# V-DETR/V-DETR

Measured on AMD Instinct MI355X. Metric: scenes/sec (train fwd+bwd) 40k-pt ScanNet, higher is better.
Workload: dtype f32

## Files before the change

v-detr_amd/csrc/attn_bwd_box4.hip:

```cpp
#include "attn_common.h"

#include <stdlib.h>

namespace vdetr {

typedef f32x4 __attribute__((may_alias)) b4_rec4_t;
typedef float __attribute__((may_alias)) b4_rec1_t;
typedef int __attribute__((may_alias)) b4_reci_t;
typedef unsigned __attribute__((may_alias)) b4_recu_t;

constexpr int kB4Waves = 16;
constexpr int kB4Threads = kB4Waves * kWave;
constexpr int kB4T = 10;
constexpr int kB4RecBytes = 64;
constexpr int kB4StripBytes = kWave * kB4RecBytes + (kWave + 4) * 4 + 2 * kWave * 4;
constexpr int kB4TableWords = 4 * kB4T * kB4T * kB4T * 4;

size_t attn_bwd_box4_lds_bytes() { return (size_t)kB4TableWords * 4 + (size_t)kB4Waves * kB4StripBytes + 64; }

__device__ __forceinline__ unsigned b4_wave_incl_scan(unsigned v) {
  v += (unsigned)__builtin_amdgcn_update_dpp(0, (int)v, 0x111, 0xF, 0xF, false);
  v += (unsigned)__builtin_amdgcn_update_dpp(0, (int)v, 0x112, 0xF, 0xF, false);
  v += (unsigned)__builtin_amdgcn_update_dpp(0, (int)v, 0x114, 0xF, 0xF, false);
  v += (unsigned)__builtin_amdgcn_update_dpp(0, (int)v, 0x118, 0xF, 0xF, false);
  v += (unsigned)__builtin_amdgcn_update_dpp(0, (int)v, kDppRowBcast15, 0xA, 0xF, false);
  v += (unsigned)__builtin_amdgcn_update_dpp(0, (int)v, kDppRowBcast31, 0xC, 0xF, false);
  return v;
}
__device__ __forceinline__ int b4_round(float x) {
  int r;
  asm("v_cvt_rpi_i32_f32 %0, %1" : "=v"(r) : "v"(x));
  return r;
}

template <bool NEAREST>
__global__ __launch_bounds__(kB4Threads) void attn_bwd_box4_kernel(AttnParams P) {
  constexpr int T = kB4T, T3 = T * T * T;
  if (P.bwd_aux[4] != 0 || P.bwd_aux[5] == 0) return;
  extern __shared__ __attribute__((aligned(16))) float smem[];
  char* lds = reinterpret_cast<char*>(smem);
  int* tab = reinterpret_cast<int*>(lds);
  const int tid = threadIdx.x, lane = tid & 63;
  const int wv = __builtin_amdgcn_readfirstlane(tid >> 6);
  char* rec = lds + (size_t)kB4TableWords * 4 + (size_t)wv * kB4StripBytes;
  char* sigs = rec + kWave * kB4RecBytes;
  char* wcnt = sigs + (kWave + 4) * 4;
  char* wfirst = wcnt + kWave * 4;
  unsigned* misc = reinterpret_cast<unsigned*>(lds + (size_t)kB4TableWords * 4 + (size_t)kB4Waves * kB4StripBytes);
  const int part = blockIdx.x & 1, nwg = gridDim.x >> 1;
  const int items = P.B * P.nQ;
  for (int i = tid; i < kB4TableWords; i += kB4Threads) tab[i] = 0;
  for (int i = lane; i < kB4StripBytes / 4; i += kWave) reinterpret_cast<b4_recu_t*>(rec)[i] = 0u;
  const int per_wg = (items + nwg - 1) / nwg;
  const int cap = bwd_query_cap(per_wg);
  float fix_scale = 1.f, fix_inv = 1.f;
  {
    const float dmax = sqrtf(__uint_as_float(P.bwd_aux[0]) * __uint_as_float(P.bwd_aux[1]));
    const float bound = 2.f * P.drop_scale * dmax * (float)cap;
    if (bound > 0.f && bound < INFINITY) {
      const int e = 30 - (int)ceilf(__log2f(bound) + 1e-3f);
      fix_scale = ldexpf(1.f, e);
      fix_inv = ldexpf(1.f, -e);
    }
  }
  unsigned* counter = const_cast<unsigned*>(P.bwd_aux) + 2 + part;
  if (tid == 0) misc[0] = atomicAdd(counter, 1u);
  __syncthreads();
  int item = (int)misc[0];
  int taken = 1;

  const int kk = lane >> 4, c15 = lane & 15;
  const int a_off = (((c15 >> 2) & 1) ^ kk) * 16 + (c15 & 3) * 4;
  const int b_offx = (2 ^ kk) * 16 + (2 * ((c15 >> 2) & 1) + (c15 >> 3)) * 4, b_offd = (3 ^ kk) * 16 + (c15 & 3) * 4;
  const int o_xi = c15 >> 3;
  const int o_lane = (((kk & 1) * T + ((c15 >> 2) & 1)) * 4 + (c15 & 3)) * 4;
  const int o_c0 = (o_xi ? 3 : 0) * T3 * 16 + o_lane, o_c1 = (o_xi ? 2 : 1) * T3 * 16 + o_lane;
  const int o_xshift = 20 + 4 * o_xi;

  using rsrc_t = __amdgpu_buffer_rsrc_t;
  auto make_rsrc = [](const void* p, unsigned bytes) {
    return __builtin_amdgcn_make_buffer_rsrc(const_cast<void*>(p), 0, (int)bytes, 0x00020000);
  };
  auto ldf = [](rsrc_t r, int voff, int soff) {
    return __builtin_bit_cast(float, __builtin_amdgcn_raw_buffer_load_b32(r, voff, soff, 0));
  };
  auto uni = [](float x) { return __int_as_float(__builtin_amdgcn_readfirstlane(__float_as_int(x))); };
  const int rowbytes = P.nK * 4;
  const bool rot = P.cos_sin != nullptr;
  const int nchunks = (P.nK + kWave - 1) / kWave;
  struct Ops { float d[4], kx, ky, kz; };
  auto fetch = [&](rsrc_t rd, rsrc_t rx, int chunk, Ops& o) {
    const int key = chunk * kWave + lane;
#pragma unroll
    for (int h = 0; h < 4; ++h)
      o.d[h] = __builtin_bit_cast(float, __builtin_amdgcn_raw_buffer_load_b32(rd, key * 4, h * rowbytes, kStreamAux));
    o.kx = ldf(rx, key * 12, 0); o.ky = ldf(rx, key * 12 + 4, 0); o.kz = ldf(rx, key * 12 + 8, 0);
  };

  int slot_of_next = 1;
  while (item < items) {
    int drawn = items;
    if (tid == 0 && taken < cap) asm volatile("global_atomic_add %0, %1, %2, off sc0\n\ts_nop 3" : "=&v"(drawn) : "v"(counter), "v"(1) : "memory");
    const int b = item / P.nQ;
    const rsrc_t rd = make_rsrc(P.dprob + (size_t)item * 4 * P.nK, 4u * rowbytes);
    const rsrc_t rx = make_rsrc(P.xyz + (size_t)b * P.nK * 3, 3u * rowbytes);
    Ops ops;
    fetch(rd, rx, wv, ops);
    const float* vp = P.vertices + (size_t)item * 24;
    const float bx0 = vp[0], bx1 = vp[6], by0 = vp[1], by1 = vp[4], bz = vp[part * 12 + 2];
    float X0 = uni(bx0), X1 = uni(bx1), Y0 = uni(by0), Y1 = uni(by1), Zp = uni(bz);
    float rc = 1.f, rs = 0.f;
    if (rot) {
      rc = uni(P.cos_sin[(size_t)item * 2]); rs = uni(P.cos_sin[(size_t)item * 2 + 1]);
      float ex = uni(vp[9]) - X0, ey = uni(vp[10]) - Y0;
      rpe_rotate(ex, ey, rc, rs);
      float fx = uni(vp[3]) - X0, fy = uni(vp[4]) - Y0;
      rpe_rotate(fx, fy, rc, rs);
      X1 = ex; Y1 = fy;
    }
    for (int chunk = wv; chunk < nchunks; chunk += kB4Waves) {
      const int ns = min(kWave, P.nK - chunk * kWave);
      const bool valid = lane < ns;
      float dx0 = X0 - ops.kx, dy0 = Y0 - ops.ky, dx1 = X1 - ops.kx, dy1 = Y1 - ops.ky;
      if (rot) {
        rpe_rotate(dx0, dy0, rc, rs);
        dx1 = dx0 + X1; dy1 = dy0 + Y1;
      }
      const AxisTap az = rpe_axis<NEAREST>(Zp - ops.kz, P);
      const AxisTap ay0 = rpe_axis<NEAREST>(dy0, P), ay1 = rpe_axis<NEAREST>(dy1, P);
      const AxisTap ax0 = rpe_axis<NEAREST>(dx0, P), ax1 = rpe_axis<NEAREST>(dx1, P);
      const int zrow = az.base * (T * T);
      const int J = (zrow + ay0.base * T) | ((zrow + ay1.base * T) << 10) | (ax0.base << 20) | (ax1.base << 24);
      const unsigned hsh = ((unsigned)J * 0x9E3779B1u) >> 26;
      const float u0 = az.wa * ay0.wa, u1 = az.wa * ay1.wa, u2 = az.wb * ay0.wa, u3 = az.wb * ay1.wa;
      const float u4 = az.wa * ay0.wb, u5 = az.wa * ay1.wb, u6 = az.wb * ay0.wb, u7 = az.wb * ay1.wb;
      const float d0 = ops.d[0] * fix_scale, d1 = ops.d[1] * fix_scale, d2 = ops.d[2] * fix_scale, d3 = ops.d[3] * fix_scale;
      if (chunk + kB4Waves < nchunks) fetch(rd, rx, chunk + kB4Waves, ops);
      __builtin_amdgcn_wave_barrier();
      unsigned rank = 0;
      if (valid) rank = __hip_atomic_fetch_add(reinterpret_cast<b4_recu_t*>(wcnt) + hsh, 1u, __ATOMIC_RELAXED, __HIP_MEMORY_SCOPE_WAVEFRONT);
      __builtin_amdgcn_wave_barrier();
      const unsigned cnt = reinterpret_cast<const b4_recu_t*>(wcnt)[lane];
      const unsigned incl = b4_wave_incl_scan(cnt);
      reinterpret_cast<b4_recu_t*>(wfirst)[lane] = incl - cnt;
      reinterpret_cast<b4_recu_t*>(wcnt)[lane] = 0u;
      __builtin_amdgcn_wave_barrier();
      if (valid) {
        const unsigned slot = reinterpret_cast<const b4_recu_t*>(wfirst)[hsh] + rank;
        char* mine = rec + slot * kB4RecBytes;
        const unsigned sw = (slot & 3u) << 4;
        *reinterpret_cast<b4_rec4_t*>(mine + sw) = f32x4{u0, u1, u2, u3};
        *reinterpret_cast<b4_rec4_t*>(mine + (sw ^ 16u)) = f32x4{u4, u5, u6, u7};
        *reinterpret_cast<b4_rec4_t*>(mine + (sw ^ 32u)) = f32x4{ax0.wa, ax1.wa, ax0.wb, ax1.wb};
        *reinterpret_cast<b4_rec4_t*>(mine + (sw ^ 48u)) = f32x4{d0, d1, d2, d3};
        reinterpret_cast<b4_reci_t*>(sigs)[slot] = J;
      }
      __builtin_amdgcn_wave_barrier();
      const int Jm = valid ? reinterpret_cast<const b4_reci_t*>(sigs)[lane] : -1;
      const int Jn = lane + 1 < ns ? reinterpret_cast<const b4_reci_t*>(sigs)[lane + 1] : -2;
      const char* rq = rec + kk * kB4RecBytes;
      float u[kWave / 4], t[kWave / 4];
#pragma unroll
      for (int i = 0; i < kWave / 4; ++i) {
        u[i] = *reinterpret_cast<const b4_rec1_t*>(rq + i * 4 * kB4RecBytes + a_off);
        t[i] = *reinterpret_cast<const b4_rec1_t*>(rq + i * 4 * kB4RecBytes + b_offx) *
               *reinterpret_cast<const b4_rec1_t*>(rq + i * 4 * kB4RecBytes + b_offd);
      }
      const unsigned long long emask = __ballot(valid && Jm != Jn);
      f32x4 acc = {0.f, 0.f, 0.f, 0.f};
      auto flush = [&](int slot) {
        const int Jg = __builtin_amdgcn_readlane(Jm, slot);
        const int cell0 = Jg & 1023, cell1 = (Jg >> 10) & 1023;
        if (lane < 32) {
          const int xb = (int)__builtin_amdgcn_ubfe((unsigned)Jg, (unsigned)o_xshift, 4u);
          char* bin0 = reinterpret_cast<char*>(tab) + ((cell0 + xb) << 4) + o_c0;
          char* bin1 = reinterpret_cast<char*>(tab) + ((cell1 + xb) << 4) + o_c1;
          atomicAdd(reinterpret_cast<int*>(bin0), b4_round(acc[0]));
          atomicAdd(reinterpret_cast<int*>(bin1), b4_round(acc[1]));
          atomicAdd(reinterpret_cast<int*>(bin0 + T * T * 16), b4_round(acc[2]));
          atomicAdd(reinterpret_cast<int*>(bin1 + T * T * 16), b4_round(acc[3]));
        }
        acc = f32x4{0.f, 0.f, 0.f, 0.f};
      };
      if (ns == kWave) {
#pragma unroll
        for (int i = 0; i < kWave / 4; ++i) {
          const unsigned eb = (unsigned)(emask >> (4 * i)) & 0xFu;
          if (eb == 0u) {
            acc = __builtin_amdgcn_mfma_f32_16x16x4f32(u[i], t[i], acc, 0, 0, 0);
          } else if (eb == 8u) {
            acc = __builtin_amdgcn_mfma_f32_16x16x4f32(u[i], t[i], acc, 0, 0, 0);
            flush(4 * i + 3);
          } else {
            const int e0 = __builtin_ctz(eb);
            const bool head = kk <= e0;
            acc = __builtin_amdgcn_mfma_f32_16x16x4f32(head ? u[i] : 0.f, t[i], acc, 0, 0, 0);
            flush(4 * i + e0);
            unsigned rest = eb & (eb - 1u);
            if ((rest & 7u) == 0u) {
              acc = __builtin_amdgcn_mfma_f32_16x16x4f32(head ? 0.f : u[i], t[i], acc, 0, 0, 0);
              if (rest) flush(4 * i + 3);
            } else {
              int s = e0 + 1;
              do {
                const int e = rest ? __builtin_ctz(rest) : 3;
                acc = __builtin_amdgcn_mfma_f32_16x16x4f32(kk >= s && kk <= e ? u[i] : 0.f, t[i], acc, 0, 0, 0);
                if (rest) {
                  flush(4 * i + e);
                  rest &= rest - 1u;
                }
                s = e + 1;
              } while (s < 4);
            }
          }
        }
      } else {
        for (int i = 0; 4 * i < ns; ++i) {
          unsigned eb = (unsigned)(emask >> (4 * i)) & 0xFu;
          const int nq = min(4, ns - 4 * i);
          const float ui = *reinterpret_cast<const b4_rec1_t*>(rq + i * 4 * kB4RecBytes + a_off);
          const float ti = *reinterpret_cast<const b4_rec1_t*>(rq + i * 4 * kB4RecBytes + b_offx) *
                           *reinterpret_cast<const b4_rec1_t*>(rq + i * 4 * kB4RecBytes + b_offd);
          int s = 0;
          do {
            const int e = eb ? __builtin_ctz(eb) : 3;
            acc = __builtin_amdgcn_mfma_f32_16x16x4f32(kk >= s && kk <= e ? ui : 0.f, ti, acc, 0, 0, 0);
            if (eb) {
              flush(4 * i + e);
              eb &= eb - 1u;
            }
            s = e + 1;
          } while (s < nq);
        }
      }
    }
    if (tid == 0) {
      asm volatile("s_waitcnt vmcnt(0)" ::: "memory");
      misc[slot_of_next] = (unsigned)drawn;
    }
    asm volatile("s_waitcnt lgkmcnt(0)\n\ts_barrier" ::: "memory");
    item = (int)misc[slot_of_next];
    slot_of_next ^= 3;
    if (taken < cap) ++taken;
  }
  __syncthreads();
  float* dst = P.dtable_part + (size_t)blockIdx.x * kB4TableWords;
  for (int i = tid; i < kB4TableWords; i += kB4Threads) dst[i] = (float)tab[i] * fix_inv;
}

int launch_attn_bwd_box4(const AttnParams& P, int grid, hipStream_t st) {
  const size_t lds = attn_bwd_box4_lds_bytes();
  if (P.rpe_nearest) {
    if (int e = set_lds(attn_bwd_box4_kernel<true>, lds, "attn_bwd_box4")) return e;
    hipLaunchKernelGGL(attn_bwd_box4_kernel<true>, dim3(grid), dim3(kB4Threads), lds, st, P);
    return check_launch("attn_bwd_box4");
  }
  if (int e = set_lds(attn_bwd_box4_kernel<false>, lds, "attn_bwd_box4")) return e;
  hipLaunchKernelGGL(attn_bwd_box4_kernel<false>, dim3(grid), dim3(kB4Threads), lds, st, P);
  return check_launch("attn_bwd_box4");
}

}
```

Baseline: 158.6.

## Split segmented MFMA reduction across accumulator halves using segment-parity masks

Uses a prefix-parity word over segment boundaries so that alternating segments are accumulated into different output halves of the 16x16 MFMA. A per-lane keep mask on the A operand routes each segment, which lets most quads run a single MFMA instead of one per segment. Flushes then come from whichever half owns the segment. This reduces the number of MFMAs and serialised branches in the full-wave path. The cost is extra bit-manipulation and more complex correctness reasoning; the partial-wave path is restricted to the lower half.

```diff
diff --git a/v-detr_amd/csrc/attn_bwd_box4.hip b/v-detr_amd/csrc/attn_bwd_box4.hip
--- a/v-detr_amd/csrc/attn_bwd_box4.hip
+++ b/v-detr_amd/csrc/attn_bwd_box4.hip
@@ -1,4 +1,5 @@
 #include "attn_common.h"
+#include "box4_walk.h"
 
 #include <stdlib.h>
 
@@ -167,11 +168,12 @@
                *reinterpret_cast<const b4_rec1_t*>(rq + i * 4 * kB4RecBytes + b_offd);
       }
       const unsigned long long emask = __ballot(valid && Jm != Jn);
+      const unsigned long long par = b4_parity_word(emask);
       f32x4 acc = {0.f, 0.f, 0.f, 0.f};
-      auto flush = [&](int slot) {
+      auto flush_half = [&](int slot, int half) {
         const int Jg = __builtin_amdgcn_readlane(Jm, slot);
         const int cell0 = Jg & 1023, cell1 = (Jg >> 10) & 1023;
-        if (lane < 32) {
+        if ((lane >> 5) == half) {
           const int xb = (int)__builtin_amdgcn_ubfe((unsigned)Jg, (unsigned)o_xshift, 4u);
           char* bin0 = reinterpret_cast<char*>(tab) + ((cell0 + xb) << 4) + o_c0;
           char* bin1 = reinterpret_cast<char*>(tab) + ((cell1 + xb) << 4) + o_c1;
@@ -179,46 +181,31 @@
           atomicAdd(reinterpret_cast<int*>(bin1), b4_round(acc[1]));
           atomicAdd(reinterpret_cast<int*>(bin0 + T * T * 16), b4_round(acc[2]));
           atomicAdd(reinterpret_cast<int*>(bin1 + T * T * 16), b4_round(acc[3]));
+          acc = f32x4{0.f, 0.f, 0.f, 0.f};
         }
-        acc = f32x4{0.f, 0.f, 0.f, 0.f};
       };
+      auto flush = [&](int slot) { flush_half(slot, b4_half_of_slot(par, slot)); };
       if (ns == kWave) {
+        const unsigned long long keep = b4_keep_word(par, c15, kk);
+        const unsigned keep_lo = (unsigned)keep, keep_hi = (unsigned)(keep >> 32);
 #pragma unroll
         for (int i = 0; i < kWave / 4; ++i) {
+          const int km = __builtin_amdgcn_sbfe((int)(i < 8 ? keep_lo : keep_hi), (unsigned)(4 * i & 31), 1u);
+          const float ua = __int_as_float(__float_as_int(u[i]) & km);
           const unsigned eb = (unsigned)(emask >> (4 * i)) & 0xFu;
-          if (eb == 0u) {
-            acc = __builtin_amdgcn_mfma_f32_16x16x4f32(u[i], t[i], acc, 0, 0, 0);
-          } else if (eb == 8u) {
-            acc = __builtin_amdgcn_mfma_f32_16x16x4f32(u[i], t[i], acc, 0, 0, 0);
-            flush(4 * i + 3);
-          } else {
-            const int e0 = __builtin_ctz(eb);
-            const bool head = kk <= e0;
-            acc = __builtin_amdgcn_mfma_f32_16x16x4f32(head ? u[i] : 0.f, t[i], acc, 0, 0, 0);
-            flush(4 * i + e0);
-            unsigned rest = eb & (eb - 1u);
-            if ((rest & 7u) == 0u) {
-              acc = __builtin_amdgcn_mfma_f32_16x16x4f32(head ? 0.f : u[i], t[i], acc, 0, 0, 0);
-              if (rest) flush(4 * i + 3);
-            } else {
-              int s = e0 + 1;
-              do {
-                const int e = rest ? __builtin_ctz(rest) : 3;
-                acc = __builtin_amdgcn_mfma_f32_16x16x4f32(kk >= s && kk <= e ? u[i] : 0.f, t[i], acc, 0, 0, 0);
-                if (rest) {
-                  flush(4 * i + e);
-                  rest &= rest - 1u;
-                }
-                s = e + 1;
-              } while (s < 4);
-            }
-          }
+          b4_walk_quad(
+              eb, 4 * i,
+              [&](int lo, int hi) {
+                const float a = (lo == 0 && hi == 3) || (kk >= lo && kk <= hi) ? ua : 0.f;
+                acc = __builtin_amdgcn_mfma_f32_16x16x4f32(a, t[i], acc, 0, 0, 0);
+              },
+              flush);
         }
       } else {
         for (int i = 0; 4 * i < ns; ++i) {
           unsigned eb = (unsigned)(emask >> (4 * i)) & 0xFu;
           const int nq = min(4, ns - 4 * i);
-          const float ui = *reinterpret_cast<const b4_rec1_t*>(rq + i * 4 * kB4RecBytes + a_off);
+          const float ui = c15 < 8 ? *reinterpret_cast<const b4_rec1_t*>(rq + i * 4 * kB4RecBytes + a_off) : 0.f;
           const float ti = *reinterpret_cast<const b4_rec1_t*>(rq + i * 4 * kB4RecBytes + b_offx) *
                            *reinterpret_cast<const b4_rec1_t*>(rq + i * 4 * kB4RecBytes + b_offd);
           int s = 0;
@@ -226,7 +213,7 @@
             const int e = eb ? __builtin_ctz(eb) : 3;
             acc = __builtin_amdgcn_mfma_f32_16x16x4f32(kk >= s && kk <= e ? ui : 0.f, ti, acc, 0, 0, 0);
             if (eb) {
-              flush(4 * i + e);
+              flush_half(4 * i + e, 0);
               eb &= eb - 1u;
             }
             s = e + 1;
diff --git a/v-detr_amd/csrc/box4_walk.h b/v-detr_amd/csrc/box4_walk.h
--- /dev/null
+++ b/v-detr_amd/csrc/box4_walk.h
@@ -0,0 +1,48 @@
+#pragma once
+
+#if defined(__HIPCC__) || defined(__CUDACC__)
+#define B4_HD __host__ __device__ __forceinline__
+#else
+#define B4_HD inline
+#endif
+
+namespace vdetr {
+
+B4_HD unsigned long long b4_parity_word(unsigned long long emask) {
+  unsigned long long x = emask << 1;
+  x ^= x << 1;
+  x ^= x << 2;
+  x ^= x << 4;
+  x ^= x << 8;
+  x ^= x << 16;
+  x ^= x << 32;
+  return x;
+}
+
+B4_HD int b4_half_of_slot(unsigned long long par, int slot) { return (int)(par >> slot) & 1; }
+
+B4_HD unsigned long long b4_keep_word(unsigned long long par, int m, int kk) { return ((m & 8) ? par : ~par) >> kk; }
+
+B4_HD int b4_quad_cut(unsigned eb) {
+  const unsigned in = eb & 7u, in2 = in & (in - 1u);
+  return in2 ? __builtin_ctz(in2) : -1;
+}
+
+template <class Mma, class Flush>
+B4_HD void b4_walk_quad(unsigned eb, int base, Mma&& mma, Flush&& flush) {
+  const int cut = b4_quad_cut(eb);
+  if (cut < 0) {
+    mma(0, 3);
+    if (eb & 7u) flush(base + __builtin_ctz(eb & 7u));
+    if (eb & 8u) flush(base + 3);
+  } else {
+    mma(0, cut);
+    flush(base + __builtin_ctz(eb));
+    flush(base + cut);
+    mma(cut + 1, 3);
+    if (cut == 1 && (eb & 4u)) flush(base + 2);
+    if (eb & 8u) flush(base + 3);
+  }
+}
+
+}
```

After: 163.4, median of 6. +3.0%, better.
